# AleoNet/snarkVM

Hardware: NVIDIA H100
Metric: bls12_377_g1_msm_points_per_sec (higher is better)
Workload: dtype u32 limbs (Montgomery integer arithmetic, IMAD pipe)

## Files before the change

snarkvm_b200/csrc/msm.cu:

```cuda
#include "msm.cuh"

#include <atomic>
#include <condition_variable>
#include <memory>
#include <mutex>
#include <utility>
#include <vector>
#include <cstdio>
#include <cstdlib>
#include <cstring>
#include <cub/device/device_scan.cuh>

#define FF_CALL_MUL 1
#include "ec.cuh"
#include "cta_inverse.cuh"
#include "quad.cuh"
#define FIELD_TEST_ENTRY test_field_op_msm
#include "testops.cuh"

namespace b200 {

static std::atomic<uint64_t> g_launches{0};
uint64_t launch_count() { return g_launches.load(); }
void count_launch(int n) { g_launches.fetch_add((uint64_t)n); }
// ... 385 lines not shown
                                                        uint32_t total_buckets, uint32_t T, uint32_t* __restrict__ prefix,
                                                        uint32_t* __restrict__ dense_out) {
    __shared__ uint4 sh_inv4[PAIR_THREADS * 3];
    uint32_t* sh_inv = reinterpret_cast<uint32_t*>(sh_inv4);
    const uint32_t total = off_out[total_buckets];
    const uint64_t o0_64 = (uint64_t)(blockIdx.x * blockDim.x + threadIdx.x) * T;
    const uint32_t o0 = o0_64 < total ? (uint32_t)o0_64 : total;
    const uint32_t o1 = (o0_64 + T < total) ? o0 + T : total;
    uint32_t lo = 0, hi = total_buckets;
    if (o0 < o1) while (hi - lo > 1) { uint32_t mid = (lo + hi) >> 1; if (off_out[mid] <= o0) lo = mid; else hi = mid; }
    uint32_t b = lo;

    Fq run = Fq::one();
    for (uint32_t o = o0; o < o1; o++) {
        while (o >= off_out[b + 1]) b++;
        const uint32_t i = o - off_out[b], base_in = off_in[b], cnt = off_in[b + 1] - base_in;
        const bool has2 = 2 * i + 1 < cnt;
        if (has2) {
            const uint32_t* pp = level_input_ptr<GATHER>(dense_bases, sorted, dense_in, base_in + 2 * i);
            const uint32_t* qp = level_input_ptr<GATHER>(dense_bases, sorted, dense_in, base_in + 2 * i + 1);
            Fq x1 = Fq::load_ldg(pp), x2 = Fq::load_ldg(qp);
            if (x1 == x2 || x1.is_zero() || x2.is_zero()) {
                DensePoint P = load_level_input<GATHER>(dense_bases, sorted, dense_in, base_in + 2 * i);
                DensePoint Q = load_level_input<GATHER>(dense_bases, sorted, dense_in, base_in + 2 * i + 1);
                Fq d;
                int kind = classify_pair(P, Q, true, d);
                if (kind >= PAIR_ADD) run = run * d;
            } else {
                run = run * (x2 - x1);
            }
        }
        run.store(prefix + (size_t)o * 12);
    }
    Fq inv = cta_shared_inverse(run, sh_inv);
    for (uint32_t o = o1; o-- > o0;) {
        while (o < off_out[b]) b--;
        const uint32_t i = o - off_out[b], base_in = off_in[b], cnt = off_in[b + 1] - base_in;
        const bool has2 = 2 * i + 1 < cnt;
        DensePoint P = load_level_input<GATHER>(dense_bases, sorted, dense_in, base_in + 2 * i);
        DensePoint Q = P;
        if (has2) Q = load_level_input<GATHER>(dense_bases, sorted, dense_in, base_in + 2 * i + 1);
        Fq d;
        int kind = classify_pair(P, Q, has2, d);
        DensePoint R;
        if (kind == PAIR_COPY1) R = P;
        else if (kind == PAIR_COPY2) R = Q;
        else if (kind == PAIR_INF) { R.inf = true; R.x = Fq::zero(); R.y = Fq::zero(); }
        else {
            Fq inv_d = (o == o0) ? inv : inv * Fq::load(prefix + (size_t)(o - 1) * 12);
            inv = inv * d;
            Fq lambda;
            if (kind == PAIR_ADD) lambda = (Q.y - P.y) * inv_d;
            else { Fq xx = P.x.sqr(); lambda = (xx.dbl() + xx) * inv_d; }
            Fq x3 = lambda.sqr() - P.x - Q.x;
            R.y = lambda * (P.x - x3) - P.y;
            R.x = x3;
            R.inf = false;
        }
        store_dense(dense_out + (size_t)o * DENSE_WORDS, R);
    }
}


FF_DEV uint32_t smem_addr_u32(const void* p) { return (uint32_t)__cvta_generic_to_shared(p); }
FF_DEV void cp_async16(uint32_t dst, const void* src) {
    asm volatile("cp.async.cg.shared.global [%0], [%1], 16;" ::"r"(dst), "l"(src) : "memory");
}
FF_DEV void cp_async_commit() { asm volatile("cp.async.commit_group;" ::: "memory"); }
FF_DEV void cp_async_wait_1() { asm volatile("cp.async.wait_group 1;" ::: "memory"); }
FF_DEV void cp_async_wait_0() { asm volatile("cp.async.wait_group 0;" ::: "memory"); }
FF_DEV void cp_async_wait_3() { asm volatile("cp.async.wait_group 3;" ::: "memory"); }

static constexpr int RING_CHUNKS = 12;
static constexpr int RING_STAGE_U4 = RING_CHUNKS * 32;
static constexpr int PAIR2_SMEM = PAIR_THREADS * 48 + 4 * 2 * RING_STAGE_U4 * 16;

FF_DEV Fq ring_fq(const uint4* slot) {
    Fq r;
#pragma unroll
    for (int i = 0; i < 3; i++) { uint4 t = slot[i * 32]; r.v[4 * i] = t.x; r.v[4 * i + 1] = t.y; r.v[4 * i + 2] = t.z; r.v[4 * i + 3] = t.w; }
    return r;
}

static constexpr uint32_t PAIR_NONE = 0xffffffffu;
template <bool GATHER>
__global__ void __launch_bounds__(256) k_pair_desc(const uint32_t* __restrict__ sorted, const uint32_t* __restrict__ off_in,
                                                   const uint32_t* __restrict__ off_out, uint32_t total_buckets, uint2* __restrict__ desc,
                                                   const uint32_t* __restrict__ in_base_ptr ) {
    const uint32_t o = blockIdx.x * blockDim.x + threadIdx.x;
    if (o >= __ldg(off_out + total_buckets)) return;
    uint32_t lo = 0, hi = total_buckets;
    while (hi - lo > 1) { uint32_t mid = (lo + hi) >> 1; if (__ldg(off_out + mid) <= o) lo = mid; else hi = mid; }
    const uint32_t i = o - __ldg(off_out + lo), base_in = __ldg(off_in + lo), cnt = __ldg(off_in + lo + 1) - base_in;
    const uint32_t idx = base_in + 2u * i;
    const bool has2 = 2u * i + 1u < cnt;
    uint2 d;
    if (GATHER) { d.x = __ldg(sorted + idx); d.y = has2 ? __ldg(sorted + idx + 1) : PAIR_NONE; }
    else { d.x = idx - (in_base_ptr ? __ldg(in_base_ptr) : 0u); d.y = has2 ? 0u : PAIR_NONE; }
    desc[o] = d;
}

struct PairDesc {
    uint32_t p, q;
    bool valid;
    FF_DEV bool has2() const { return valid && q != PAIR_NONE; }
};
FF_DEV PairDesc pair_load_desc(int64_t j, uint32_t nv, const uint2* __restrict__ dlane) {
    PairDesc d; d.p = 0; d.q = PAIR_NONE; d.valid = false;
    if (j < 0 || j >= (int64_t)nv) return d;
    const uint2 v = __ldg(dlane + 32 * j);
    d.p = v.x; d.q = v.y; d.valid = true;
    return d;
}
template <bool GATHER>
FF_DEV const uint32_t* pair_src(const PairDesc& d, int which, const uint32_t* __restrict__ records, uint32_t in_words) {
    if (GATHER) return records + (size_t)((which ? d.q : d.p) & 0x7fffffffu) * BASE_WORDS;
    return records + (size_t)(d.p + (uint32_t)which) * in_words;
}
template <bool GATHER, bool FULL>
FF_DEV void pair_issue(const PairDesc& d, uint4* ring, int st, int lane, const uint32_t* __restrict__ records, uint32_t in_words, int chunks) {
    if (d.valid) {
        const uint32_t dst = smem_addr_u32(ring + (size_t)st * (size_t)(chunks * 32) + lane);
        const uint32_t* p = pair_src<GATHER>(d, 0, records, in_words);
#pragma unroll
        for (int k = 0; k < (FULL ? 6 : 3); k++) cp_async16(dst + (uint32_t)k * 512u, p + 4 * k);
        if (d.q != PAIR_NONE) {
            const uint32_t* q = pair_src<GATHER>(d, 1, records, in_words);
#pragma unroll
            for (int k = 0; k < (FULL ? 6 : 3); k++) cp_async16(dst + (uint32_t)((FULL ? 6 : 3) + k) * 512u, q + 4 * k);
        }
    }
    cp_async_commit();
}
template <bool GATHER>
FF_DEV int pair_classify_global(const PairDesc& d, const uint32_t* __restrict__ records, uint32_t in_words, Fq& den) {
    DensePoint P = load_dense(pair_src<GATHER>(d, 0, records, in_words));
    DensePoint Q = load_dense(pair_src<GATHER>(d, 1, records, in_words));
    if (GATHER) { if ((d.p >> 31) && !P.inf) P.y = P.y.neg(); if ((d.q >> 31) && !Q.inf) Q.y = Q.y.neg(); }
    return classify_pair(P, Q, true, den);
}

template <bool GATHER, int MINB>
__global__ void __launch_bounds__(PAIR_THREADS, MINB) k_pair_level2(const uint32_t* __restrict__ records ,
                                                         uint32_t in_words, const uint2* __restrict__ desc, const uint32_t* __restrict__ total_ptr,
                                                         uint32_t T_bound, uint32_t* __restrict__ prefix, uint32_t* __restrict__ dense_out,
                                                         uint32_t* __restrict__ sm_slots) {
    (void)T_bound;
    extern __shared__ uint4 pair2_smem[];
    __shared__ uint32_t sh_slot;
    uint32_t* sh_inv = reinterpret_cast<uint32_t*>(pair2_smem);
    const int lane = threadIdx.x & 31, warp = threadIdx.x >> 5;
    uint4* ring = pair2_smem + PAIR_THREADS * 3 + (size_t)warp * 2 * RING_STAGE_U4;
    if (threadIdx.x == 0) {
        uint32_t smid;
        asm volatile("mov.u32 %0, %%smid;" : "=r"(smid));
        sh_slot = atomicAdd(sm_slots + (smid & 255u), 1u);
    }
    __syncthreads();
    const int inv_warp = (int)(sh_slot & 3u);
    const uint32_t total = __ldg(total_ptr);
    const uint64_t lanes = (uint64_t)gridDim.x * PAIR_THREADS;
    const uint32_t T = total > lanes ? (uint32_t)((total + lanes - 1) / lanes) : 1u;
    const uint64_t w0_64 = ((uint64_t)blockIdx.x * (PAIR_THREADS / 32) + (uint32_t)warp) * 32ull * T + (uint32_t)lane;
    uint32_t nv = 0;
    if (w0_64 < total) { const uint64_t left = (total - w0_64 + 31) / 32; nv = left < T ? (uint32_t)left : T; }
    const uint2* dlane = desc + w0_64;
    uint32_t* plane = prefix + w0_64 * 12;
    uint32_t* olane = dense_out + w0_64 * DENSE_WORDS;

    Fq run = Fq::one();
    {
        constexpr int PF = 3;
        PairDesc q0 = pair_load_desc(0, nv, dlane), q1 = pair_load_desc(1, nv, dlane), q2 = pair_load_desc(2, nv, dlane);
        pair_issue<GATHER, false>(q0, ring, 0, lane, records, in_words, 6);
        pair_issue<GATHER, false>(q1, ring, 1, lane, records, in_words, 6);
        pair_issue<GATHER, false>(q2, ring, 2, lane, records, in_words, 6);
        PairDesc ahead = pair_load_desc(PF, nv, dlane);
        for (uint32_t j = 0; j < T; j++) {
            pair_issue<GATHER, false>(ahead, ring, (int)((j + PF) & 3u), lane, records, in_words, 6);
            const PairDesc cur = q0;
            q0 = q1; q1 = q2; q2 = ahead;
            ahead = pair_load_desc((int64_t)j + PF + 1, nv, dlane);
            cp_async_wait_3();
            Fq d = Fq::one();
            if (cur.has2()) {
                const uint4* slot_p = ring + (size_t)(j & 3u) * (6 * 32) + lane;
                Fq x1 = ring_fq(slot_p), x2 = ring_fq(slot_p + 3 * 32);
                if (x1 == x2 || x1.is_zero() || x2.is_zero()) {
                    Fq den;
                    if (pair_classify_global<GATHER>(cur, records, in_words, den) >= PAIR_ADD) d = den;
                } else {
                    d = x2 - x1;
                }
            }
            run = run * d;
            if (cur.valid) run.store(plane + (size_t)j * (32 * 12));
        }
        cp_async_wait_0();
    }
    Fq inv = cta_shared_inverse_by(run, sh_inv, inv_warp);
    {
        PairDesc cur = pair_load_desc((int64_t)T - 1, nv, dlane);
        pair_issue<GATHER, true>(cur, ring, 0, lane, records, in_words, 12);
        PairDesc nxt = pair_load_desc((int64_t)T - 2, nv, dlane);
        for (uint32_t k = 0; k < T; k++) {
            const uint32_t j = T - 1 - k;
            pair_issue<GATHER, true>(nxt, ring, (int)((k + 1) & 1u), lane, records, in_words, 12);
            PairDesc nn = pair_load_desc((int64_t)j - 2, nv, dlane);
            Fq pf = Fq::one();
            if (cur.valid && j != 0) pf = Fq::load(plane + (size_t)(j - 1) * (32 * 12));
            cp_async_wait_1();
            const uint4* slot_p = ring + (size_t)(k & 1u) * RING_STAGE_U4 + lane;
            int kind = PAIR_COPY1;
            Fq d = Fq::one(), num = Fq::zero();
            const bool has2 = cur.has2();
            const bool negP = GATHER && (cur.p >> 31), negQ = GATHER && has2 && (cur.q >> 31);
            if (has2) {
                Fq x1 = ring_fq(slot_p), x2 = ring_fq(slot_p + 6 * 32);
                if (x1 == x2 || x1.is_zero() || x2.is_zero()) {
                    DensePoint P, Q;
                    P.x = x1; P.y = ring_fq(slot_p + 3 * 32); P.inf = P.x.is_zero() && P.y.is_zero();
                    Q.x = x2; Q.y = ring_fq(slot_p + 9 * 32); Q.inf = Q.x.is_zero() && Q.y.is_zero();
                    if (negP && !P.inf) P.y = P.y.neg();
                    if (negQ && !Q.inf) Q.y = Q.y.neg();
                    Fq den;
                    kind = classify_pair(P, Q, true, den);
                    if (kind >= PAIR_ADD) d = den;
                    if (kind == PAIR_ADD) num = Q.y - P.y;
                    else if (kind == PAIR_DBL) { Fq xx = P.x.sqr(); num = xx.dbl() + xx; }
                } else {
                    kind = PAIR_ADD;
                    d = x2 - x1;
                    Fq y1 = ring_fq(slot_p + 3 * 32), y2 = ring_fq(slot_p + 9 * 32);
                    if (negP == negQ) { num = y2 - y1; if (negP) num = num.neg(); }
                    else { num = y2 + y1; if (negQ) num = num.neg(); }
                }
            }
            Fq inv_next = inv * d;
            Fq inv_d = (j != 0) ? inv * pf : inv;
            inv = inv_next;
            Fq lambda = num * inv_d;
            Fq x3 = lambda.sqr();
            {
                Fq x1 = ring_fq(slot_p), x2 = has2 ? ring_fq(slot_p + 6 * 32) : x1;
                x3 = x3 - x1 - x2;
                Fq t = x1 - x3;
                Fq y3 = lambda * t;
                if (cur.valid) {
                    DensePoint R;
                    if (kind >= PAIR_ADD) {
                        Fq y1 = ring_fq(slot_p + 3 * 32);
                        R.x = x3; R.y = negP ? y3 + y1 : y3 - y1; R.inf = false;
                    } else if (kind == PAIR_INF) {
                        R.inf = true; R.x = Fq::zero(); R.y = Fq::zero();
                    } else {
                        const int c0 = (kind == PAIR_COPY2) ? 6 : 0;
                        R.x = ring_fq(slot_p + c0 * 32); R.y = ring_fq(slot_p + (c0 + 3) * 32);
                        R.inf = R.x.is_zero() && R.y.is_zero();
                        if (((kind == PAIR_COPY2) ? negQ : negP) && !R.inf) R.y = R.y.neg();
                    }
                    store_dense(olane + (size_t)j * (32 * DENSE_WORDS), R);
                }
            }
            cur = nxt; nxt = nn;
        }
        cp_async_wait_0();
    }
}

__global__ void k_halve_counts(const uint32_t* __restrict__ off_in, uint32_t* __restrict__ cnt_out, uint32_t total_buckets) {
    uint32_t i = blockIdx.x * blockDim.x + threadIdx.x;
    if (i < total_buckets) cnt_out[i] = (off_in[i + 1] - off_in[i] + 1u) >> 1;
    else if (i == total_buckets) cnt_out[i] = 0;
}
__global__ void k_items_from_offsets(const uint32_t* __restrict__ off, uint32_t* __restrict__ items, uint32_t total_buckets, uint32_t cap,
                                     uint32_t* __restrict__ hot, uint32_t hot_max, uint32_t keep) {
    uint32_t i = blockIdx.x * blockDim.x + threadIdx.x;
    if (i < total_buckets) {
        const uint32_t it = (off[i + 1] - off[i] + cap - 1u) / cap;
        items[i] = it;
        if (hot != nullptr && it > keep) { const uint32_t pos = atomicAdd(hot, 1u); if (pos < hot_max) hot[1u + pos] = i; }
    } else if (i == total_buckets) items[i] = 0;
}

__global__ void __launch_bounds__(MSM_ACC_THREADS, MSM_ACC_MINBLOCKS) k_bucket_accumulate_dense(
    const uint32_t* __restrict__ dense, const uint32_t* __restrict__ bucket_start, const uint32_t* __restrict__ item_start,
    uint32_t total_buckets, uint32_t cap, uint32_t* __restrict__ partial) {
    uint32_t t = blockIdx.x * blockDim.x + threadIdx.x;
    uint32_t total_items = item_start[total_buckets];
    if (t >= total_items) return;
    uint32_t lo = 0, hi = total_buckets;
    while (hi - lo > 1) { uint32_t mid = (lo + hi) >> 1; if (item_start[mid] <= t) lo = mid; else hi = mid; }
    uint32_t wb = lo, seg = t - item_start[wb];
    uint32_t b0 = bucket_start[wb], b1 = bucket_start[wb + 1];
    uint32_t s0 = b0 + seg * cap, s1 = s0 + cap < b1 ? s0 + cap : b1;
    XYZZ acc = XYZZ::infinity();
    DensePoint p = load_dense(dense + (size_t)s0 * DENSE_WORDS);
    for (uint32_t k = s0; k < s1; k++) {
        AffinePoint cur; cur.x = p.x; cur.y = p.y; cur.inf = p.inf;
        if (k + 1 < s1) p = load_dense(dense + (size_t)(k + 1) * DENSE_WORDS);
        acc.add_affine(cur, false);
    }
    acc.store(partial + (size_t)t * XYZZ_WORDS);
}

__global__ void k_group_counts(const uint32_t* __restrict__ start_in, uint32_t* __restrict__ cnt_out, uint32_t total_buckets) {
    uint32_t i = blockIdx.x * blockDim.x + threadIdx.x;
    if (i < total_buckets) cnt_out[i] = (start_in[i + 1] - start_in[i] + 31u) >> 5;
    else if (i == total_buckets) cnt_out[i] = 0;
}
__global__ void __launch_bounds__(128) k_partial_group_sum(const uint32_t* __restrict__ partial_in, const uint32_t* __restrict__ start_in,
                                                            const uint32_t* __restrict__ start_out, uint32_t total_buckets,
                                                            uint32_t* __restrict__ partial_out) {
    uint32_t t = blockIdx.x * blockDim.x + threadIdx.x;
    if (t >= start_out[total_buckets]) return;
    uint32_t lo = 0, hi = total_buckets;
    while (hi - lo > 1) { uint32_t mid = (lo + hi) >> 1; if (start_out[mid] <= t) lo = mid; else hi = mid; }
    uint32_t g = t - start_out[lo];
    uint32_t i0 = start_in[lo] + g * 32u, i1 = start_in[lo + 1];
    if (i0 + 32u < i1) i1 = i0 + 32u;
    XYZZ s = XYZZ::load(partial_in + (size_t)i0 * XYZZ_WORDS);
    for (uint32_t i = i0 + 1; i < i1; i++) s.add(XYZZ::load(partial_in + (size_t)i * XYZZ_WORDS));
    s.store(partial_out + (size_t)t * XYZZ_WORDS);
}

FF_DEV uint32_t fold_rounds_of(uint32_t cnt, uint32_t& final_cnt, uint32_t keep = 32u) {
    uint32_t r = 0;
    while (cnt > keep) { cnt = (cnt + 31u) >> 5; r++; }
    final_cnt = cnt;
    return r;
}

FF_DEV XYZZ bucket_sum(const uint32_t* __restrict__ partial, const uint32_t* __restrict__ item_start, uint32_t wb) {
    uint32_t i0 = item_start[wb], i1 = item_start[wb + 1];
    XYZZ s = XYZZ::infinity();
    for (uint32_t i = i0; i < i1; i++) {
        if (i == i0) s = XYZZ::load(partial + (size_t)i * XYZZ_WORDS);
        else s.add(XYZZ::load(partial + (size_t)i * XYZZ_WORDS));
    }
    return s;
}

struct SetOffsets {
    uint32_t set0, per_job, top_first, nbuckets;
    FF_DEV uint32_t of(uint32_t set) const {
        const uint32_t s = (set0 + set) % per_job;
        return s > top_first ? (s - top_first) * nbuckets : 0u;
    }
};
static SetOffsets set_offsets(const MsmPlan& plan, bool flat, uint32_t set0) {
    if (flat) return SetOffsets{0u, 1u, 0u, 0u};
    return SetOffsets{set0, (uint32_t)plan.nsets, (uint32_t)plan.nwin - 1u, plan.nbuckets};
}

template <bool PAIRS>
__global__ void __launch_bounds__(128) k_bucket_reduce(const uint32_t* __restrict__ partial, const uint32_t* __restrict__ item_start,
                                                        uint32_t nbuckets, uint32_t chunk, uint32_t chunks_per_window,
                                                        uint32_t nwin, uint32_t* __restrict__ out,
                                                        const uint32_t* __restrict__ partial_b = nullptr, int folds = 0,
                                                        SetOffsets so = SetOffsets{0u, 1u, 0u, 0u}) {
    uint32_t t = blockIdx.x * blockDim.x + threadIdx.x;
    if (t >= chunks_per_window * nwin) return;
    uint32_t w = t / chunks_per_window, j = t % chunks_per_window;
    uint32_t lo = j * chunk, hi = lo + chunk;
    XYZZ running = XYZZ::infinity(), acc = XYZZ::infinity();
    for (uint32_t b = hi; b-- > lo;) {
        XYZZ s;
        if (PAIRS && folds > 0) {
            const uint32_t wb = w * nbuckets + b, i0 = item_start[wb];
            uint32_t cnt = item_start[wb + 1] - i0;
            const uint32_t r = fold_rounds_of(cnt, cnt, 1u);
            s = cnt ? XYZZ::load(((r & 1u) ? partial_b : partial) + (size_t)i0 * XYZZ_WORDS) : XYZZ::infinity();
        } else
            s = bucket_sum(partial, item_start, w * nbuckets + b);
        running.add(s);
        acc.add(running);
// ... 515 lines not shown
    const uint32_t nwins = (uint32_t)njobs * wins_per_job;
    uint32_t gu = nwins;
    if (levels > 0) {
        size_t per_win = set_cap * (size_t)(records ? 84 + 4 * rec_words : 104) + 1;
        size_t fit = budget / per_win;
        if (fit < 1) fit = 1;
        if (fit < gu) {
            const uint32_t ngroups = (uint32_t)((nwins + fit - 1) / fit);
            gu = (nwins + ngroups - 1) / ngroups;
        }
    }
    auto set_of = [&](uint32_t u) { return (u / wins_per_job) * sets_per_job + u % wins_per_job; };
    uint32_t gw = 0;
    for (uint32_t u0 = 0; u0 < nwins; u0 += gu) {
        const uint32_t s = set_of(u0 + (nwins - u0 < gu ? nwins - u0 : gu)) - set_of(u0);
        if (s > gw) gw = s;
    }
    const uint32_t TBg = gw * plan.nbuckets;
    size_t entries_g = set_cap * (size_t)gu;
    if (entries_g > max_entries) entries_g = max_entries;
    if (records && entries_g >= 0x7fffffffull) return (int)cudaErrorInvalidValue;
    bool warp_reduce = plan.nbuckets <= 1024u;
    bool acc_g8 = levels == 0 && max_entries <= 100000;
    int quad_path = 1;
    if (const char* e = getenv("SNARKVM_B200_MSM_QUAD")) quad_path = atoi(e);
    bool acc_q8 = quad_path != 0 && warp_reduce && levels == 0 && (size_t)TB + max_entries / 32 <= 1100;
    if (const char* e = getenv("SNARKVM_B200_MSM_WARP_PATH")) { if (atoi(e) == 0) { warp_reduce = false; acc_g8 = false; acc_q8 = false; } }
    bool quad_tail_large = true;
    if (plan.nbuckets < 16384u) quad_tail_large = false;
    if (const char* e = getenv("SNARKVM_B200_MSM_QUAD_TAIL")) quad_tail_large = atoi(e) != 0;
    const bool quad_fold = quad_path != 0 && warp_reduce && levels == 0;
    const bool large_hot = quad_path != 0 && quad_tail_large && !warp_reduce;
    const uint32_t hot_keep = large_hot ? 1u : 32u;
    if (acc_q8) acc_g8 = false;
    uint32_t item_cap = plan.cap;
    if (acc_g8) {
        size_t per_lane = max_entries / 300000 + 1;
        if (per_lane < 4) per_lane = 4;
        if (per_lane > 16) per_lane = 16;
        item_cap = (uint32_t)per_lane * 8u;
        if (const char* e = getenv("SNARKVM_B200_MSM_CAP")) { long v = atol(e); if (v >= 1) item_cap = (uint32_t)v; }
    }
    if (acc_q8) {
        size_t cap16 = ((set_cap + 15) / 16 + 7) & ~(size_t)7;
        item_cap = (uint32_t)(cap16 < 32 ? 32 : cap16);
    } else if (quad_fold && !acc_g8 && max_entries <= 900000) {
        item_cap = max_entries <= 150000 ? 4 : 8;
        if (const char* e = getenv("SNARKVM_B200_MSM_CAP")) { long v = atol(e); if (v >= 1) item_cap = (uint32_t)v; }
    }
    const bool small_cap = quad_fold && !acc_g8 && !acc_q8 && item_cap != plan.cap;
    const size_t max_items = (size_t)TBg + entries_g / (item_cap < plan.cap ? item_cap : plan.cap) + 1;
    const size_t hot_max = max_items / 2 + 1;
    const size_t dense_cap_a = entries_g / 2 + TBg + 1, dense_cap_b = entries_g / 4 + 2 * (size_t)TBg + 1;

    size_t pair_waves = 0;
    if (const char* e = getenv("SNARKVM_B200_MSM_PAIR_WAVES")) { long v = atol(e); if (v >= 1) pair_waves = (size_t)v; }
    bool pair_v1 = false;
    if (const char* e = getenv("SNARKVM_B200_MSM_PAIR_V1")) pair_v1 = atoi(e) != 0;
    int pair_minb = 4;
    if (const char* e = getenv("SNARKVM_B200_MSM_PAIR_MINB")) { int v = atoi(e); if (v == 3 || v == 4) pair_minb = v; }
    int sm_count = 0;
    {
        static std::once_flag smem_once[64];
        int dev = 0; cudaGetDevice(&dev);
        std::call_once(smem_once[dev & 63], [] {
            cudaFuncSetAttribute(k_pair_level2<true, 4>, cudaFuncAttributeMaxDynamicSharedMemorySize, PAIR2_SMEM);
            cudaFuncSetAttribute(k_pair_level2<false, 4>, cudaFuncAttributeMaxDynamicSharedMemorySize, PAIR2_SMEM);
            cudaFuncSetAttribute(k_pair_level2<true, 3>, cudaFuncAttributeMaxDynamicSharedMemorySize, PAIR2_SMEM);
            cudaFuncSetAttribute(k_pair_level2<false, 3>, cudaFuncAttributeMaxDynamicSharedMemorySize, PAIR2_SMEM);
        });
        const cudaError_t e = cudaDeviceGetAttribute(&sm_count, cudaDevAttrMultiProcessorCount, dev);
        if (e != cudaSuccess) return (int)e;
    }
    const uint32_t chunk = plan.nbuckets < 16u ? plan.nbuckets : 16u;
    const uint32_t tree = 8;
    const uint32_t chunks_per_set = plan.nbuckets / chunk;

    size_t cub_bytes = 0;
    if (cub::DeviceScan::ExclusiveSum(nullptr, cub_bytes, (uint32_t*)nullptr, (uint32_t*)nullptr, (int)(TB + 1), stream) != cudaSuccess) return (int)cudaErrorUnknown;
    if (cub_bytes < 16) cub_bytes = 16;

    uint32_t *hist, *bucket_start, *cursors, *items, *item_start, *items2, *sorted, *partial, *partial2, *red_a, *red_b;
    uint32_t *off_a = nullptr, *off_b = nullptr, *dense_a = nullptr, *dense_b = nullptr, *prefix = nullptr, *dense_bases = nullptr, *sm_slots = nullptr;
    uint32_t *dense0 = nullptr, *cnt_tmp = nullptr, *hot_dev = nullptr;
    uint2* desc = nullptr;
    uint8_t* cub_tmp;
    Arena ar;
    auto layout = [&](Arena& a) {
        hist = a.take<uint32_t>((size_t)TB + 1);
        bucket_start = a.take<uint32_t>((size_t)TB + 1);
        cursors = a.take<uint32_t>((size_t)TB + 1);
        items = a.take<uint32_t>((size_t)TBg + 1);
        item_start = a.take<uint32_t>((size_t)TBg + 1);
        items2 = a.take<uint32_t>((size_t)TBg + 1);
        sorted = records ? nullptr : a.take<uint32_t>(max_entries);
        cnt_tmp = a.take<uint32_t>((size_t)TBg + 1);
        partial = a.take<uint32_t>(max_items * XYZZ_WORDS);
        partial2 = a.take<uint32_t>(((quad_fold || large_hot) ? max_items : (size_t)TBg + max_items / 32 + 2) * XYZZ_WORDS);
        hot_dev = a.take<uint32_t>(hot_max + 2);
        red_a = a.take<uint32_t>((size_t)gw * (2 * chunks_per_set > 2 * ((plan.nbuckets + 7u) / 8u) ? 2 * chunks_per_set : 2 * ((plan.nbuckets + 7u) / 8u)) * XYZZ_WORDS);
        red_b = a.take<uint32_t>((size_t)gw * (chunks_per_set / tree + 1 > 2 * ((plan.nbuckets + 63u) / 64u) + 2 ? chunks_per_set / tree + 1 : 2 * ((plan.nbuckets + 63u) / 64u) + 2) * XYZZ_WORDS);
        cub_tmp = a.take<uint8_t>(cub_bytes);
        if (!flat && !records) dense_bases = a.take<uint32_t>(total_bases * (size_t)BASE_WORDS);
        if (records) dense0 = a.take<uint32_t>(entries_g * (size_t)rec_words);
        if (levels > 0) {
            off_a = a.take<uint32_t>((size_t)TBg + 1);
            off_b = a.take<uint32_t>((size_t)TBg + 1);
            dense_a = a.take<uint32_t>(dense_cap_a * DENSE_WORDS);
            if (levels > 1) dense_b = records && dense_cap_b * DENSE_WORDS <= entries_g * (size_t)rec_words ? dense0 : a.take<uint32_t>(dense_cap_b * DENSE_WORDS);
            prefix = a.take<uint32_t>(dense_cap_a * 12);
            desc = a.take<uint2>(dense_cap_a);
            sm_slots = a.take<uint32_t>(256);
        }
    };
    layout(ar);
    const size_t scratch_bytes = ar.off;
    void* block = nullptr;
    DeviceScratch* ds = nullptr;
    if ((rc = scratch_acquire(&block, scratch_bytes, stream, &ds)) != 0) return rc;
    ar.base = (uint8_t*)block; ar.off = 0;
    layout(ar);

    CUDA_TRY(cudaMemsetAsync(hist, 0, (size_t)(TB + 1) * 4, stream));
    if (sm_slots) CUDA_TRY(cudaMemsetAsync(sm_slots, 0, 256 * 4, stream));
    if (quad_fold) CUDA_TRY(cudaMemsetAsync(hot_dev, 0, 4, stream));
    {
        {
            ProfScope sort_scope(PROF_MSM_SORT, stream);
            for (int pass = 0; pass < (records ? 1 : 2); pass++) {
                for (int i = 0; i < nsegs; i++) {
                    const MsmSegment& sg = segs[i];
                    if (sg.n == 0) continue;
                    const unsigned grid = (unsigned)((sg.n + 255) / 256);
                    const uint32_t slot_base = sg.job * sets_per_job * plan.nbuckets;
                    const uint32_t* sc = (const uint32_t*)sg.d_scalars;
                    const size_t fl = flat ? table_n : 0;
                    if (pass == 0) {
                        if (sg.mont) k_digits<false, true><<<grid, 256, 0, stream>>>(sc, sg.n, plan.c, plan.c_top, plan.nwin, plan.nbuckets, hist, nullptr, fl, slot_base, sg.base0, d_flags);
                        else k_digits<false, false><<<grid, 256, 0, stream>>>(sc, sg.n, plan.c, plan.c_top, plan.nwin, plan.nbuckets, hist, nullptr, fl, slot_base, sg.base0, d_flags);
                    } else {
                        if (sg.mont) k_digits<true, true><<<grid, 256, 0, stream>>>(sc, sg.n, plan.c, plan.c_top, plan.nwin, plan.nbuckets, cursors, sorted, fl, slot_base, sg.base0, d_flags);
                        else k_digits<true, false><<<grid, 256, 0, stream>>>(sc, sg.n, plan.c, plan.c_top, plan.nwin, plan.nbuckets, cursors, sorted, fl, slot_base, sg.base0, d_flags);
                    }
                    count_launch();
                }
                if (pass == 0) {
                    CUDA_TRY(cub::DeviceScan::ExclusiveSum(cub_tmp, cub_bytes, hist, bucket_start, (int)(TB + 1), stream));
                    CUDA_TRY(cudaMemcpyAsync(cursors, bucket_start, (size_t)(TB + 1) * 4, cudaMemcpyDeviceToDevice, stream));
                    count_launch(2);
                }
            }
        }
        const uint32_t* gather_src = flat ? table : dense_bases;
        if (!flat && !records) {
            ProfScope acc_scope(PROF_MSM_ACCUMULATE, stream);
            size_t at = 0;
            for (int i = 0; i < nbases; i++) {
                if (bases[i].n == 0) continue;
                k_densify_bases<<<(unsigned)((bases[i].n + 255) / 256), 256, 0, stream>>>((const uint8_t*)bases[i].d_points, bases[i].stride, bases[i].n,
                                                                                        dense_bases + at * BASE_WORDS);
                count_launch();
                at += bases[i].n;
            }
        }
        for (uint32_t u0 = 0; u0 < nwins; u0 += gu) {
            const uint32_t un = nwins - u0 < gu ? nwins - u0 : gu;
            const uint32_t w0 = set_of(u0), wn = set_of(u0 + un) - w0;
            const uint32_t tb = wn * plan.nbuckets;
            const uint32_t* bs = bucket_start + (size_t)w0 * plan.nbuckets;
            const SetOffsets so = set_offsets(plan, flat, w0);
            size_t entries = set_cap * (size_t)un;
            if (entries > max_entries) entries = max_entries;
            if (large_hot) CUDA_TRY(cudaMemsetAsync(hot_dev, 0, 4, stream));
            size_t items_bound = 1;
            size_t items_launched = 1;
            const uint32_t* final_partial = nullptr;
            const uint32_t* final_start = nullptr;
            if (levels == 0) {
                const uint32_t cap = (acc_g8 || acc_q8 || small_cap) ? item_cap : plan.cap;
                k_items_per_bucket<<<(tb + 256) / 256, 256, 0, stream>>>(hist + (size_t)w0 * plan.nbuckets, items, tb, cap, (quad_fold || large_hot) ? hot_dev : nullptr, (uint32_t)hot_max, hot_keep);
                CUDA_TRY(cub::DeviceScan::ExclusiveSum(cub_tmp, cub_bytes, items, item_start, (int)(tb + 1), stream));
                count_launch(2);
                const size_t group_items = (size_t)tb + entries / cap + 1;
                items_bound = set_cap / cap + 1;
                items_launched = group_items;
                ProfScope acc_scope(PROF_MSM_ACCUMULATE, stream);
                if (acc_q8) {
                    k_bucket_accumulate_q8<<<(unsigned)((group_items * 32 + 127) / 128), 128, 0, stream>>>(gather_src, sorted, bs, item_start, tb, cap, partial);
                    items_bound = 1;
                } else if (acc_g8)
                    k_bucket_accumulate_g8<<<(unsigned)((group_items * ACC_G + 127) / 128), 128, 0, stream>>>(gather_src, sorted, bs, item_start, tb, cap, partial);
                else
                    k_bucket_accumulate<<<(unsigned)((group_items + MSM_ACC_THREADS - 1) / MSM_ACC_THREADS), MSM_ACC_THREADS, 0, stream>>>(
                        gather_src, sorted, bs, item_start, tb, cap, partial);
                count_launch();
            } else {
                if (records) {
                    ProfScope sort_scope(PROF_MSM_SORT, stream);
                    for (int i = 0; i < nsegs; i++) {
                        const MsmSegment& sg = segs[i];
                        if (sg.n == 0) continue;
                        const int64_t first = (int64_t)sg.job * wins_per_job;
                        int w_lo, w_hi;
                        if (flat) {
                            if (first < (int64_t)u0 || first >= (int64_t)u0 + un) continue;
                            w_lo = 0; w_hi = plan.nwin;
                        } else {
                            const int64_t lo_w = (int64_t)u0 - first, hi_w = (int64_t)u0 + un - first;
                            w_lo = lo_w < 0 ? 0 : (int)lo_w; w_hi = hi_w > plan.nwin ? plan.nwin : (int)hi_w;
                            if (w_lo >= w_hi) continue;
                        }
                        const unsigned grid = (unsigned)((sg.n + 255) / 256);
                        const uint32_t slot_base = sg.job * sets_per_job * plan.nbuckets;
                        const uint32_t* sc = (const uint32_t*)sg.d_scalars;
                        const int ct = plan.c_top, nw = plan.nwin;
                        if (flat) {
                            if (sg.mont) k_scatter_records<true, true><<<grid, 256, 0, stream>>>(sc, sg.n, nullptr, 0, table, table_n, plan.c, ct, nw, plan.nbuckets, cursors, slot_base, w_lo, w_hi, bs, (uint4*)dense0, rec_words);
                            else k_scatter_records<false, true><<<grid, 256, 0, stream>>>(sc, sg.n, nullptr, 0, table, table_n, plan.c, ct, nw, plan.nbuckets, cursors, slot_base, w_lo, w_hi, bs, (uint4*)dense0, rec_words);
                        } else {
                            if (sg.mont) k_scatter_records<true, false><<<grid, 256, 0, stream>>>(sc, sg.n, seg_points[i], seg_stride[i], nullptr, 0, plan.c, ct, nw, plan.nbuckets, cursors, slot_base, w_lo, w_hi, bs, (uint4*)dense0, rec_words);
                            else k_scatter_records<false, false><<<grid, 256, 0, stream>>>(sc, sg.n, seg_points[i], seg_stride[i], nullptr, 0, plan.c, ct, nw, plan.nbuckets, cursors, slot_base, w_lo, w_hi, bs, (uint4*)dense0, rec_words);
                        }
                        count_launch();
                    }
                }
                ProfScope acc_scope(PROF_MSM_ACCUMULATE, stream);
                const uint32_t* off_in = bs;
                uint32_t* off_bufs[2] = {off_a, off_b};
                uint32_t* dense_bufs[2] = {dense_a, dense_b};
                const uint32_t* dense_in = records ? dense0 : nullptr;
                size_t bound = entries;
                for (int l = 0; l < levels; l++) {
                    uint32_t* off_out = off_bufs[l & 1];
                    uint32_t* dense_out = dense_bufs[l & 1];
                    k_halve_counts<<<(tb + 256) / 256, 256, 0, stream>>>(off_in, cnt_tmp, tb);
                    CUDA_TRY(cub::DeviceScan::ExclusiveSum(cub_tmp, cub_bytes, cnt_tmp, off_out, (int)(tb + 1), stream));
                    bound = bound / 2 + tb;
                    const size_t wave = (size_t)sm_count * (pair_v1 ? 4 : pair_minb) * 128;
                    size_t waves = (bound + 1024 * wave - 1) / (1024 * wave);
                    if (pair_waves) waves = pair_waves;
                    size_t T = (bound + waves * wave - 1) / (waves * wave);
                    const size_t nthreads = (bound + T - 1) / T;
                    const unsigned lgrid = (unsigned)((nthreads + 127) / 128);
                    if (pair_v1) {
                        if (l == 0 && !records)
                            k_pair_level<true><<<lgrid, 128, 0, stream>>>(gather_src, sorted, nullptr, off_in, off_out, tb, (uint32_t)T, prefix, dense_out);
                        else
                            k_pair_level<false><<<lgrid, 128, 0, stream>>>(nullptr, nullptr, dense_in, off_in, off_out, tb, (uint32_t)T, prefix, dense_out);
                    } else {
                        const unsigned dgrid = (unsigned)((bound + 255) / 256);
                        if (l == 0 && !records) {
                            k_pair_desc<true><<<dgrid, 256, 0, stream>>>(sorted, off_in, off_out, tb, desc, nullptr);
                            if (pair_minb == 3) k_pair_level2<true, 3><<<lgrid, 128, PAIR2_SMEM, stream>>>(gather_src, BASE_WORDS, desc, off_out + tb, (uint32_t)T, prefix, dense_out, sm_slots);
                            else k_pair_level2<true, 4><<<lgrid, 128, PAIR2_SMEM, stream>>>(gather_src, BASE_WORDS, desc, off_out + tb, (uint32_t)T, prefix, dense_out, sm_slots);
                        } else {
                            k_pair_desc<false><<<dgrid, 256, 0, stream>>>(nullptr, off_in, off_out, tb, desc, l == 0 ? bs : nullptr);
                            const uint32_t in_words = l == 0 ? rec_words : (uint32_t)DENSE_WORDS;
                            if (pair_minb == 3) k_pair_level2<false, 3><<<lgrid, 128, PAIR2_SMEM, stream>>>(dense_in, in_words, desc, off_out + tb, (uint32_t)T, prefix, dense_out, sm_slots);
                            else k_pair_level2<false, 4><<<lgrid, 128, PAIR2_SMEM, stream>>>(dense_in, in_words, desc, off_out + tb, (uint32_t)T, prefix, dense_out, sm_slots);
                        }
                        count_launch(1);
                    }
                    count_launch(3);
                    off_in = off_out;
                    dense_in = dense_out;
                }
                k_items_from_offsets<<<(tb + 256) / 256, 256, 0, stream>>>(off_in, items, tb, plan.cap, large_hot ? hot_dev : nullptr, (uint32_t)hot_max, hot_keep);
                CUDA_TRY(cub::DeviceScan::ExclusiveSum(cub_tmp, cub_bytes, items, item_start, (int)(tb + 1), stream));
                const size_t group_items = (size_t)tb + bound / plan.cap + 1;
                items_bound = ((set_cap >> levels) + 1) / plan.cap + 1;
                items_launched = group_items;
                k_bucket_accumulate_dense<<<(unsigned)((group_items + MSM_ACC_THREADS - 1) / MSM_ACC_THREADS), MSM_ACC_THREADS, 0, stream>>>(
                    dense_in, off_in, item_start, tb, plan.cap, partial);
                count_launch(3);
            }
            ProfScope red_scope(PROF_MSM_REDUCE, stream);
            int quad_rounds = 0;
            if (quad_fold) {
                size_t worst = acc_q8 ? 1 : items_bound;
                const uint32_t* p_in = partial; uint32_t* p_out = partial2;
                while (worst > 32) {
                    k_fold_hot_quad<<<(unsigned)sm_count * 8, 128, 0, stream>>>(p_in, item_start, hot_dev, (uint32_t)hot_max, (uint32_t)quad_rounds, 32u, p_out);
                    count_launch();
                    worst = (worst + 31) / 32;
                    quad_rounds++;
                    const uint32_t* t1 = p_in; p_in = p_out; p_out = (uint32_t*)t1;
                }
                final_partial = partial; final_start = item_start;
            } else if (large_hot) {
                size_t worst = items_bound;
                const uint32_t* p_in = partial; uint32_t* p_out = partial2;
                while (worst > 1) {
                    k_fold_hot_quad<<<(unsigned)sm_count * 8, 128, 0, stream>>>(p_in, item_start, hot_dev, (uint32_t)hot_max, (uint32_t)quad_rounds, 1u, p_out);
                    count_launch();
                    worst = (worst + 31) / 32;
                    quad_rounds++;
                    const uint32_t* t1 = p_in; p_in = p_out; p_out = (uint32_t*)t1;
                }
                final_partial = partial; final_start = item_start;
            } else {
                size_t worst = items_bound;
                size_t total_bound = items_launched;
                uint32_t* p_in = partial; uint32_t* p_out = partial2;
                uint32_t* st_in = item_start; uint32_t* st_out = items2;
                while (worst > 1) {
                    k_group_counts<<<(tb + 256) / 256, 256, 0, stream>>>(st_in, cnt_tmp, tb);
                    CUDA_TRY(cub::DeviceScan::ExclusiveSum(cub_tmp, cub_bytes, cnt_tmp, st_out, (int)(tb + 1), stream));
                    const size_t out_bound = (size_t)tb + total_bound / 32 + 1;
                    total_bound = out_bound;
                    k_partial_group_sum<<<(unsigned)((out_bound + 127) / 128), 128, 0, stream>>>(p_in, st_in, st_out, tb, p_out);
                    count_launch(3);
                    worst = (worst + 31) / 32;
                    uint32_t* t1 = p_in; p_in = p_out; p_out = t1;
                    uint32_t* t2 = st_in; st_in = st_out; st_out = t2;
                }
                final_partial = p_in; final_start = st_in;
            }
            uint32_t* group_sums = d_window_sums + (size_t)w0 * XYZZ_WORDS;
            if (warp_reduce && quad_path != 0) {
                const uint32_t qchunks = (plan.nbuckets + 7u) / 8u;
                k_bucket_reduce_quad<<<(wn * qchunks * 32u + 127u) / 128u, 128, 0, stream>>>(final_partial, quad_fold ? partial2 : final_partial, final_start,
                                                                                              quad_rounds, plan.nbuckets, qchunks, wn, red_a);
                const uint32_t* ent = red_a;
                uint32_t m = qchunks;
                int lgw = 3;
                if (m > 64u) {
                    const uint32_t groups = (m + 7u) / 8u;
                    k_combine_level_quad<<<(wn * groups * 32u + 127u) / 128u, 128, 0, stream>>>(ent, m, wn, lgw, red_b);
                    count_launch();
                    ent = red_b; m = groups; lgw += 3;
                }
                k_window_combine_quad<<<wn, 32u * ((m + 7u) / 8u), 0, stream>>>(ent, m, lgw, group_sums, so);
                count_launch(2);
                continue;
            }
            if (warp_reduce) {
                const uint32_t wchunks = (plan.nbuckets + 31u) / 32u;
                k_bucket_reduce_warp<<<(wn * wchunks * 32u + 127u) / 128u, 128, 0, stream>>>(final_partial, final_start, plan.nbuckets, wchunks, wn, red_a);
                k_window_combine_warp<<<wn, 32, 0, stream>>>(red_a, wchunks, group_sums, so);
                count_launch(2);
                continue;
            }
            const uint32_t nthreads = chunks_per_set * wn;
            if (quad_path != 0 && quad_tail_large) {
// ... 375 lines not shown
```

Measured before the change: 169.8 million.

## Handle odd-bucket singletons in descriptor kernel, pair only full pairs

The descriptor kernel now copies the leftover single point of each odd-sized bucket straight to the output. The pair-level kernel then processes only true pairs, scattering results through a per-pair output position, so lanes no longer waste the batched-inversion pipeline on singleton copies. Bucket lookup in the descriptor and accumulate kernels switches from per-thread binary search to a warp-cooperative walk over offsets. The cost is an extra CUB scan, an extra out_pos buffer and scattered writes instead of coalesced per-lane stores.

```diff
diff --git a/snarkvm_b200/csrc/msm.cu b/snarkvm_b200/csrc/msm.cu
--- a/snarkvm_b200/csrc/msm.cu
+++ b/snarkvm_b200/csrc/msm.cu
@@ -491,34 +491,88 @@
     return r;
 }
 
-static constexpr uint32_t PAIR_NONE = 0xffffffffu;
+FF_DEV uint32_t warp_bucket_first(const uint32_t* __restrict__ off, uint32_t nb, uint32_t x) {
+    uint32_t lo = 0, hi = nb;
+    while (hi - lo > 1) { const uint32_t mid = (lo + hi) >> 1; if (__ldg(off + mid) <= x) lo = mid; else hi = mid; }
+    return lo;
+}
+FF_DEV uint32_t warp_bucket_walk(const uint32_t* __restrict__ off, uint32_t nb, uint32_t b, uint32_t x) {
+    const int lane = threadIdx.x & 31;
+    uint32_t res = b;
+    bool done = false;
+    for (int round = 0;; round++) {
+        const uint32_t k = b + 1u + (uint32_t)lane;
+        const uint32_t e = k <= nb ? __ldg(off + k) : 0xffffffffu;
+        uint32_t c = 0;
+#pragma unroll
+        for (uint32_t s = 16; s >= 1; s >>= 1)
+            if (__shfl_sync(0xffffffffu, e, (int)(c + s - 1u)) <= x) c += s;
+        const uint32_t e31 = __shfl_sync(0xffffffffu, e, 31);
+        if (!done && e31 > x) { res = b + c; done = true; }
+        if (__all_sync(0xffffffffu, done)) return res;
+        b += 32u;
+        if (round == 1) break;
+    }
+    if (!done) { uint32_t lo = b, hi = nb; while (hi - lo > 1) { const uint32_t mid = (lo + hi) >> 1; if (__ldg(off + mid) <= x) lo = mid; else hi = mid; } res = lo; }
+    return res;
+}
+
+static constexpr int DESC_CHUNKS = 8;
 template <bool GATHER>
 __global__ void __launch_bounds__(256) k_pair_desc(const uint32_t* __restrict__ sorted, const uint32_t* __restrict__ off_in,
-                                                   const uint32_t* __restrict__ off_out, uint32_t total_buckets, uint2* __restrict__ desc,
-                                                   const uint32_t* __restrict__ in_base_ptr ) {
-    const uint32_t o = blockIdx.x * blockDim.x + threadIdx.x;
-    if (o >= __ldg(off_out + total_buckets)) return;
-    uint32_t lo = 0, hi = total_buckets;
-    while (hi - lo > 1) { uint32_t mid = (lo + hi) >> 1; if (__ldg(off_out + mid) <= o) lo = mid; else hi = mid; }
-    const uint32_t i = o - __ldg(off_out + lo), base_in = __ldg(off_in + lo), cnt = __ldg(off_in + lo + 1) - base_in;
-    const uint32_t idx = base_in + 2u * i;
-    const bool has2 = 2u * i + 1u < cnt;
-    uint2 d;
-    if (GATHER) { d.x = __ldg(sorted + idx); d.y = has2 ? __ldg(sorted + idx + 1) : PAIR_NONE; }
-    else { d.x = idx - (in_base_ptr ? __ldg(in_base_ptr) : 0u); d.y = has2 ? 0u : PAIR_NONE; }
-    desc[o] = d;
+                                                   const uint32_t* __restrict__ off_out, const uint32_t* __restrict__ pair_off,
+                                                   uint32_t total_buckets, uint2* __restrict__ desc, uint32_t* __restrict__ out_pos,
+                                                   const uint32_t* __restrict__ in_base_ptr ,
+                                                   const uint32_t* __restrict__ records, uint32_t in_words, uint32_t* __restrict__ dense_out) {
+    const uint32_t t = blockIdx.x * blockDim.x + threadIdx.x;
+    const uint32_t in_base = (!GATHER && in_base_ptr) ? __ldg(in_base_ptr) : 0u;
+    if (t < total_buckets) {
+        const uint32_t end = __ldg(off_in + t + 1);
+        if ((end - __ldg(off_in + t)) & 1u) {
+            const uint32_t idx = end - 1u;
+            DensePoint P;
+            if (GATHER) {
+                const uint32_t s = __ldg(sorted + idx);
+                P = load_dense(records + (size_t)(s & 0x7fffffffu) * BASE_WORDS);
+                if ((s >> 31) && !P.inf) P.y = P.y.neg();
+            } else {
+                P = load_dense(records + (size_t)(idx - in_base) * in_words);
+            }
+            store_dense(dense_out + (size_t)(__ldg(off_out + t + 1) - 1u) * DENSE_WORDS, P);
+        }
+    }
+    const uint32_t total = __ldg(pair_off + total_buckets);
+    const uint32_t lane = threadIdx.x & 31u;
+    const uint64_t j0_64 = (uint64_t)(t >> 5) * (32u * DESC_CHUNKS);
+    if (j0_64 >= total) return;
+    uint32_t j0 = (uint32_t)j0_64;
+    uint32_t b = warp_bucket_first(pair_off, total_buckets, j0);
+    for (int c = 0; c < DESC_CHUNKS && j0 < total; c++, j0 += 32u) {
+        const uint32_t j = j0 + lane < total ? j0 + lane : total - 1u;
+        const uint32_t bj = warp_bucket_walk(pair_off, total_buckets, b, j);
+        b = __shfl_sync(0xffffffffu, bj, 31);
+        if (j0 + lane < total) {
+            const uint32_t i = j - __ldg(pair_off + bj);
+            const uint32_t idx = __ldg(off_in + bj) + 2u * i, o = __ldg(off_out + bj) + i;
+            uint2 d;
+            if (GATHER) { d.x = __ldg(sorted + idx); d.y = __ldg(sorted + idx + 1); out_pos[j] = o; }
+            else { d.x = idx - in_base; d.y = o; }
+            desc[j] = d;
+        }
+    }
 }
 
 struct PairDesc {
-    uint32_t p, q;
+    uint32_t p, q, o;
     bool valid;
-    FF_DEV bool has2() const { return valid && q != PAIR_NONE; }
 };
-FF_DEV PairDesc pair_load_desc(int64_t j, uint32_t nv, const uint2* __restrict__ dlane) {
-    PairDesc d; d.p = 0; d.q = PAIR_NONE; d.valid = false;
+template <bool GATHER, bool POS>
+FF_DEV PairDesc pair_load_desc(int64_t j, uint32_t nv, const uint2* __restrict__ dlane, const uint32_t* __restrict__ olane) {
+    PairDesc d; d.p = 0; d.q = 0; d.o = 0; d.valid = false;
     if (j < 0 || j >= (int64_t)nv) return d;
     const uint2 v = __ldg(dlane + 32 * j);
     d.p = v.x; d.q = v.y; d.valid = true;
+    if (POS) d.o = GATHER ? __ldg(olane + 32 * j) : v.y;
     return d;
 }
 template <bool GATHER>
@@ -533,11 +587,9 @@
         const uint32_t* p = pair_src<GATHER>(d, 0, records, in_words);
 #pragma unroll
         for (int k = 0; k < (FULL ? 6 : 3); k++) cp_async16(dst + (uint32_t)k * 512u, p + 4 * k);
-        if (d.q != PAIR_NONE) {
-            const uint32_t* q = pair_src<GATHER>(d, 1, records, in_words);
-#pragma unroll
-            for (int k = 0; k < (FULL ? 6 : 3); k++) cp_async16(dst + (uint32_t)((FULL ? 6 : 3) + k) * 512u, q + 4 * k);
-        }
+        const uint32_t* q = pair_src<GATHER>(d, 1, records, in_words);
+#pragma unroll
+        for (int k = 0; k < (FULL ? 6 : 3); k++) cp_async16(dst + (uint32_t)((FULL ? 6 : 3) + k) * 512u, q + 4 * k);
     }
     cp_async_commit();
 }
@@ -551,7 +603,8 @@
 
 template <bool GATHER, int MINB>
 __global__ void __launch_bounds__(PAIR_THREADS, MINB) k_pair_level2(const uint32_t* __restrict__ records ,
-                                                         uint32_t in_words, const uint2* __restrict__ desc, const uint32_t* __restrict__ total_ptr,
+                                                         uint32_t in_words, const uint2* __restrict__ desc, const uint32_t* __restrict__ out_pos,
+                                                         const uint32_t* __restrict__ total_ptr,
                                                          uint32_t T_bound, uint32_t* __restrict__ prefix, uint32_t* __restrict__ dense_out,
                                                          uint32_t* __restrict__ sm_slots) {
     (void)T_bound;
@@ -574,25 +627,26 @@
     uint32_t nv = 0;
     if (w0_64 < total) { const uint64_t left = (total - w0_64 + 31) / 32; nv = left < T ? (uint32_t)left : T; }
     const uint2* dlane = desc + w0_64;
+    const uint32_t* poslane = GATHER ? out_pos + w0_64 : nullptr;
     uint32_t* plane = prefix + w0_64 * 12;
-    uint32_t* olane = dense_out + w0_64 * DENSE_WORDS;
 
     Fq run = Fq::one();
     {
         constexpr int PF = 3;
-        PairDesc q0 = pair_load_desc(0, nv, dlane), q1 = pair_load_desc(1, nv, dlane), q2 = pair_load_desc(2, nv, dlane);
+        PairDesc q0 = pair_load_desc<GATHER, false>(0, nv, dlane, poslane), q1 = pair_load_desc<GATHER, false>(1, nv, dlane, poslane),
+                 q2 = pair_load_desc<GATHER, false>(2, nv, dlane, poslane);
         pair_issue<GATHER, false>(q0, ring, 0, lane, records, in_words, 6);
         pair_issue<GATHER, false>(q1, ring, 1, lane, records, in_words, 6);
         pair_issue<GATHER, false>(q2, ring, 2, lane, records, in_words, 6);
-        PairDesc ahead = pair_load_desc(PF, nv, dlane);
+        PairDesc ahead = pair_load_desc<GATHER, false>(PF, nv, dlane, poslane);
         for (uint32_t j = 0; j < T; j++) {
             pair_issue<GATHER, false>(ahead, ring, (int)((j + PF) & 3u), lane, records, in_words, 6);
             const PairDesc cur = q0;
             q0 = q1; q1 = q2; q2 = ahead;
-            ahead = pair_load_desc((int64_t)j + PF + 1, nv, dlane);
+            ahead = pair_load_desc<GATHER, false>((int64_t)j + PF + 1, nv, dlane, poslane);
             cp_async_wait_3();
             Fq d = Fq::one();
-            if (cur.has2()) {
+            if (cur.valid) {
                 const uint4* slot_p = ring + (size_t)(j & 3u) * (6 * 32) + lane;
                 Fq x1 = ring_fq(slot_p), x2 = ring_fq(slot_p + 3 * 32);
                 if (x1 == x2 || x1.is_zero() || x2.is_zero()) {
@@ -609,22 +663,21 @@
     }
     Fq inv = cta_shared_inverse_by(run, sh_inv, inv_warp);
     {
-        PairDesc cur = pair_load_desc((int64_t)T - 1, nv, dlane);
+        PairDesc cur = pair_load_desc<GATHER, true>((int64_t)T - 1, nv, dlane, poslane);
         pair_issue<GATHER, true>(cur, ring, 0, lane, records, in_words, 12);
-        PairDesc nxt = pair_load_desc((int64_t)T - 2, nv, dlane);
+        PairDesc nxt = pair_load_desc<GATHER, true>((int64_t)T - 2, nv, dlane, poslane);
         for (uint32_t k = 0; k < T; k++) {
             const uint32_t j = T - 1 - k;
             pair_issue<GATHER, true>(nxt, ring, (int)((k + 1) & 1u), lane, records, in_words, 12);
-            PairDesc nn = pair_load_desc((int64_t)j - 2, nv, dlane);
+            PairDesc nn = pair_load_desc<GATHER, true>((int64_t)j - 2, nv, dlane, poslane);
             Fq pf = Fq::one();
             if (cur.valid && j != 0) pf = Fq::load(plane + (size_t)(j - 1) * (32 * 12));
             cp_async_wait_1();
             const uint4* slot_p = ring + (size_t)(k & 1u) * RING_STAGE_U4 + lane;
             int kind = PAIR_COPY1;
             Fq d = Fq::one(), num = Fq::zero();
-            const bool has2 = cur.has2();
-            const bool negP = GATHER && (cur.p >> 31), negQ = GATHER && has2 && (cur.q >> 31);
-            if (has2) {
+            const bool negP = GATHER && (cur.p >> 31), negQ = GATHER && (cur.q >> 31);
+            if (cur.valid) {
                 Fq x1 = ring_fq(slot_p), x2 = ring_fq(slot_p + 6 * 32);
                 if (x1 == x2 || x1.is_zero() || x2.is_zero()) {
                     DensePoint P, Q;
@@ -651,7 +704,7 @@
             Fq lambda = num * inv_d;
             Fq x3 = lambda.sqr();
             {
-                Fq x1 = ring_fq(slot_p), x2 = has2 ? ring_fq(slot_p + 6 * 32) : x1;
+                Fq x1 = ring_fq(slot_p), x2 = ring_fq(slot_p + 6 * 32);
                 x3 = x3 - x1 - x2;
                 Fq t = x1 - x3;
                 Fq y3 = lambda * t;
@@ -668,7 +721,7 @@
                         R.inf = R.x.is_zero() && R.y.is_zero();
                         if (((kind == PAIR_COPY2) ? negQ : negP) && !R.inf) R.y = R.y.neg();
                     }
-                    store_dense(olane + (size_t)j * (32 * DENSE_WORDS), R);
+                    store_dense(dense_out + (size_t)cur.o * DENSE_WORDS, R);
                 }
             }
             cur = nxt; nxt = nn;
@@ -677,10 +730,11 @@
     }
 }
 
-__global__ void k_halve_counts(const uint32_t* __restrict__ off_in, uint32_t* __restrict__ cnt_out, uint32_t total_buckets) {
+__global__ void k_halve_counts(const uint32_t* __restrict__ off_in, uint32_t* __restrict__ cnt_out, uint32_t* __restrict__ pairs_out,
+                               uint32_t total_buckets) {
     uint32_t i = blockIdx.x * blockDim.x + threadIdx.x;
-    if (i < total_buckets) cnt_out[i] = (off_in[i + 1] - off_in[i] + 1u) >> 1;
-    else if (i == total_buckets) cnt_out[i] = 0;
+    if (i < total_buckets) { const uint32_t c = off_in[i + 1] - off_in[i]; cnt_out[i] = (c + 1u) >> 1; pairs_out[i] = c >> 1; }
+    else if (i == total_buckets) { cnt_out[i] = 0; pairs_out[i] = 0; }
 }
 __global__ void k_items_from_offsets(const uint32_t* __restrict__ off, uint32_t* __restrict__ items, uint32_t total_buckets, uint32_t cap,
                                      uint32_t* __restrict__ hot, uint32_t hot_max, uint32_t keep) {
@@ -697,10 +751,12 @@
     uint32_t total_buckets, uint32_t cap, uint32_t* __restrict__ partial) {
     uint32_t t = blockIdx.x * blockDim.x + threadIdx.x;
     uint32_t total_items = item_start[total_buckets];
+    const uint32_t t0 = t & ~31u;
+    if (t0 >= total_items) return;
+    const uint32_t wb = warp_bucket_walk(item_start, total_buckets, warp_bucket_first(item_start, total_buckets, t0),
+                                         t < total_items ? t : total_items - 1u);
     if (t >= total_items) return;
-    uint32_t lo = 0, hi = total_buckets;
-    while (hi - lo > 1) { uint32_t mid = (lo + hi) >> 1; if (item_start[mid] <= t) lo = mid; else hi = mid; }
-    uint32_t wb = lo, seg = t - item_start[wb];
+    uint32_t seg = t - item_start[wb];
     uint32_t b0 = bucket_start[wb], b1 = bucket_start[wb + 1];
     uint32_t s0 = b0 + seg * cap, s1 = s0 + cap < b1 ? s0 + cap : b1;
     XYZZ acc = XYZZ::infinity();
@@ -1382,7 +1438,7 @@
 
     uint32_t *hist, *bucket_start, *cursors, *items, *item_start, *items2, *sorted, *partial, *partial2, *red_a, *red_b;
     uint32_t *off_a = nullptr, *off_b = nullptr, *dense_a = nullptr, *dense_b = nullptr, *prefix = nullptr, *dense_bases = nullptr, *sm_slots = nullptr;
-    uint32_t *dense0 = nullptr, *cnt_tmp = nullptr, *hot_dev = nullptr;
+    uint32_t *dense0 = nullptr, *cnt_tmp = nullptr, *hot_dev = nullptr, *pair_cnt = nullptr, *pair_off = nullptr, *out_pos = nullptr;
     uint2* desc = nullptr;
     uint8_t* cub_tmp;
     Arena ar;
@@ -1410,6 +1466,9 @@
             if (levels > 1) dense_b = records && dense_cap_b * DENSE_WORDS <= entries_g * (size_t)rec_words ? dense0 : a.take<uint32_t>(dense_cap_b * DENSE_WORDS);
             prefix = a.take<uint32_t>(dense_cap_a * 12);
             desc = a.take<uint2>(dense_cap_a);
+            if (!records) out_pos = a.take<uint32_t>(dense_cap_a);
+            pair_cnt = a.take<uint32_t>((size_t)TBg + 1);
+            pair_off = a.take<uint32_t>((size_t)TBg + 1);
             sm_slots = a.take<uint32_t>(256);
         }
     };
@@ -1533,14 +1592,18 @@
                 for (int l = 0; l < levels; l++) {
                     uint32_t* off_out = off_bufs[l & 1];
                     uint32_t* dense_out = dense_bufs[l & 1];
-                    k_halve_counts<<<(tb + 256) / 256, 256, 0, stream>>>(off_in, cnt_tmp, tb);
+                    k_halve_counts<<<(tb + 256) / 256, 256, 0, stream>>>(off_in, cnt_tmp, pair_cnt, tb);
                     CUDA_TRY(cub::DeviceScan::ExclusiveSum(cub_tmp, cub_bytes, cnt_tmp, off_out, (int)(tb + 1), stream));
+                    if (!pair_v1) CUDA_TRY(cub::DeviceScan::ExclusiveSum(cub_tmp, cub_bytes, pair_cnt, pair_off, (int)(tb + 1), stream));
+                    const size_t pair_bound = pair_v1 ? bound / 2 + tb : bound / 2;
                     bound = bound / 2 + tb;
                     const size_t wave = (size_t)sm_count * (pair_v1 ? 4 : pair_minb) * 128;
-                    size_t waves = (bound + 1024 * wave - 1) / (1024 * wave);
+                    size_t waves = (pair_bound + 1024 * wave - 1) / (1024 * wave);
                     if (pair_waves) waves = pair_waves;
-                    size_t T = (bound + waves * wave - 1) / (waves * wave);
-                    const size_t nthreads = (bound + T - 1) / T;
+                    if (waves == 0) waves = 1;
+                    size_t T = (pair_bound + waves * wave - 1) / (waves * wave);
+                    if (T == 0) T = 1;
+                    const size_t nthreads = pair_bound > T ? (pair_bound + T - 1) / T : 1;
                     const unsigned lgrid = (unsigned)((nthreads + 127) / 128);
                     if (pair_v1) {
                         if (l == 0 && !records)
@@ -1548,18 +1611,21 @@
                         else
                             k_pair_level<false><<<lgrid, 128, 0, stream>>>(nullptr, nullptr, dense_in, off_in, off_out, tb, (uint32_t)T, prefix, dense_out);
                     } else {
-                        const unsigned dgrid = (unsigned)((bound + 255) / 256);
+                        const size_t desc_warps = (pair_bound + 32 * DESC_CHUNKS - 1) / (32 * DESC_CHUNKS);
+                        const size_t desc_threads = desc_warps * 32 > (size_t)tb ? desc_warps * 32 : (size_t)tb;
+                        const unsigned dgrid = (unsigned)((desc_threads + 255) / 256);
+                        const uint32_t* pair_total = pair_off + tb;
                         if (l == 0 && !records) {
-                            k_pair_desc<true><<<dgrid, 256, 0, stream>>>(sorted, off_in, off_out, tb, desc, nullptr);
-                            if (pair_minb == 3) k_pair_level2<true, 3><<<lgrid, 128, PAIR2_SMEM, stream>>>(gather_src, BASE_WORDS, desc, off_out + tb, (uint32_t)T, prefix, dense_out, sm_slots);
-                            else k_pair_level2<true, 4><<<lgrid, 128, PAIR2_SMEM, stream>>>(gather_src, BASE_WORDS, desc, off_out + tb, (uint32_t)T, prefix, dense_out, sm_slots);
+                            k_pair_desc<true><<<dgrid, 256, 0, stream>>>(sorted, off_in, off_out, pair_off, tb, desc, out_pos, nullptr, gather_src, BASE_WORDS, dense_out);
+                            if (pair_minb == 3) k_pair_level2<true, 3><<<lgrid, 128, PAIR2_SMEM, stream>>>(gather_src, BASE_WORDS, desc, out_pos, pair_total, (uint32_t)T, prefix, dense_out, sm_slots);
+                            else k_pair_level2<true, 4><<<lgrid, 128, PAIR2_SMEM, stream>>>(gather_src, BASE_WORDS, desc, out_pos, pair_total, (uint32_t)T, prefix, dense_out, sm_slots);
                         } else {
-                            k_pair_desc<false><<<dgrid, 256, 0, stream>>>(nullptr, off_in, off_out, tb, desc, l == 0 ? bs : nullptr);
                             const uint32_t in_words = l == 0 ? rec_words : (uint32_t)DENSE_WORDS;
-                            if (pair_minb == 3) k_pair_level2<false, 3><<<lgrid, 128, PAIR2_SMEM, stream>>>(dense_in, in_words, desc, off_out + tb, (uint32_t)T, prefix, dense_out, sm_slots);
-                            else k_pair_level2<false, 4><<<lgrid, 128, PAIR2_SMEM, stream>>>(dense_in, in_words, desc, off_out + tb, (uint32_t)T, prefix, dense_out, sm_slots);
+                            k_pair_desc<false><<<dgrid, 256, 0, stream>>>(nullptr, off_in, off_out, pair_off, tb, desc, nullptr, l == 0 ? bs : nullptr, dense_in, in_words, dense_out);
+                            if (pair_minb == 3) k_pair_level2<false, 3><<<lgrid, 128, PAIR2_SMEM, stream>>>(dense_in, in_words, desc, nullptr, pair_total, (uint32_t)T, prefix, dense_out, sm_slots);
+                            else k_pair_level2<false, 4><<<lgrid, 128, PAIR2_SMEM, stream>>>(dense_in, in_words, desc, nullptr, pair_total, (uint32_t)T, prefix, dense_out, sm_slots);
                         }
-                        count_launch(1);
+                        count_launch(2);
                     }
                     count_launch(3);
                     off_in = off_out;
```

After: 175.9 million, median of 6. +3.6%, better.
